# UzL-ITS/dash

Measured on AMD Instinct MI355X. Metric: online garbled inferences/sec (MiniONN CIFAR-10 CNN), higher is better.
Workload: dtype uint8 label components / int8 MFMA (exact modular arithmetic)

## Files before the change

dash_amd/csrc/hip/kernels_gadget.hip:

```cpp
#include <cmath>
#include <cstdio>
#include <cstdlib>

#include "gadget_common.h"

namespace dash {
namespace dev {


template <int TM>
__device__ __forceinline__ void approx_casts_out(const AesCtx& aes, const SignArgs& a, const ModC* mc, int j, int b,
                                                 int64_t e, const u128 (&P)[TM], const u128* TA, uint32_t col, u128 H) {
    const int64_t N = a.N;
    const int t = a.t;
    u128* out = a.mrsP + (static_cast<int64_t>(b) * a.crt.k + j) * t * N + e;
    if (a.fused) {
#pragma unroll
        for (int d = 0; d < TM; ++d)
            if (d < t) out[static_cast<int64_t>(d) * N] = P[d];
        for (int d = TM; d < t; ++d) out[static_cast<int64_t>(d) * N] = TA[col * t + d] - H;
        return;
    }
    const u128* T1 = a.cast1 + (static_cast<int64_t>(b) * N + e) * a.n_cast;
    out[0] = P[0];
// ... 1032 lines not shown
#pragma unroll
            for (int u = 0; u < kChunk; ++u)
                if (i0 + kChunk + u < n) nxt[u] = L[static_cast<int64_t>(i0 + kChunk + u) * N];
#pragma unroll
            for (int u = 0; u < kChunk; ++u)
                if (i0 + u < n) {
                    const uint32_t g = sg.next(m);
                    const uint32_t ev = se.next(m);
                    Y[static_cast<int64_t>(i0 + u) * N] =
                        static_cast<act_t>(modq(ev + ypr * static_cast<uint32_t>(cur[u]) + static_cast<uint32_t>(p) - g, m));
                }
#pragma unroll
            for (int u = 0; u < kChunk; ++u) cur[u] = nxt[u];
        }
    }
}

constexpr int kRroBS = 256;
__global__ __launch_bounds__(kRroBS) void k_rescale_relu_out_s(MrsArgs a, SignArgs sa, Act x, Act y, const u128* gtab,
                                                                const u128* etab, const ModC* mc, const uint32_t* te0,
                                                                const uint32_t* rk) {
    (void)te0;
    (void)rk;
    __shared__ __attribute__((aligned(16))) uint8_t stg[128 * kRroBS];
    const int j = blockIdx.y, b = blockIdx.z;
    const int64_t N = a.N;
    const int k = a.crt.k;
    const int p = a.crt.p[j];
    const ModC m = mc[p];
    const int n = static_cast<int>(m.n);
    const int tid = static_cast<int>(threadIdx.x);
    const uint32_t inv = static_cast<uint32_t>(a.sinv[j]);
    act_t* L = x.p[j] + static_cast<int64_t>(b) * n * N;
    act_t* Y = y.p[j] + static_cast<int64_t>(b) * n * N;
    for (int64_t e0 = static_cast<int64_t>(blockIdx.x) * kRroBS; e0 < N; e0 += static_cast<int64_t>(gridDim.x) * kRroBS) {
        const int64_t e = min(e0 + tid, N - 1);
        const int64_t be = static_cast<int64_t>(b) * N + e;
        const int64_t bke = (static_cast<int64_t>(b) * k + j) * N + e;
        const u128 HS = a.ys[(static_cast<int64_t>(b) * a.ny + j) * N + e];
        const u128 HM = a.ys[(static_cast<int64_t>(b) * a.ny + k + j / 8) * N + e] >> (16 * (j % 8));
        const uint32_t cS = a.cs[be];
        const u128* E3 = etab + (be * k + j) * 3;
        const u128 Eraw = E3[cS];
        const u128 mini = E3[2];
        const u128* grow = gtab + be * sa.crt.sum + sa.crt.prefix[j];
        const u128 P = a.pf[bke];
        __syncthreads();
        if (j != 0) lds_stage_rows<kRroBS, 4>(stg, L, N, e0, 0, n);
        __syncthreads();
        DigitStream s;
        s.init(P);
        CompressFwd cf;
        cf.init();
        u128 Graw = 0;
        constexpr int kRroG = 8;
        if (j == 0 && m.bits == 1) {
            Graw = grow[static_cast<uint32_t>(P) & 1u];
#pragma unroll
            for (int w = 0; w < 4; ++w) {
                const uint32_t pw = static_cast<uint32_t>(P >> (32 * w));
#pragma unroll 8
                for (int u = 0; u < 32; ++u) {
                    const int c = 32 * w + u;
                    if (c >= n) break;
                    stg[c * kRroBS + tid] = static_cast<uint8_t>((pw >> u) & 1u);
                }
            }
        }
        for (int c0 = 0; c0 < ((j == 0 && m.bits == 1) ? 0 : n); c0 += kRroG) {
            uint32_t w8[kRroG];
#pragma unroll
            for (int u = 0; u < kRroG; ++u) w8[u] = (j != 0 && c0 + u < n) ? stg[(c0 + u) * kRroBS + tid] : 0u;
#pragma unroll
            for (int u = 0; u < kRroG; ++u) {
                const int c = c0 + u;
                if (c >= n) break;
                const uint32_t v = j == 0 ? s.next(m) : modq(w8[u] * inv + s.next(m), m);
                if (c == 0) Graw = grow[v];
                stg[c * kRroBS + tid] = static_cast<uint8_t>(v);
                if (j != 0) cf.push(v, m);
            }
        }
        const u128 key = j == 0 ? P : cf.finish();
        __syncthreads();
        lds_store_rows<kRroBS>(L, stg, N, e0, 0, n);
        const u128 G = Graw - hard_pad(key, a.rgate0 ^ static_cast<uint64_t>(e), tw_sub(kTwMmg, j), 0);
        const u128 E = Eraw - HS;
        const int16_t t16 = static_cast<int16_t>(static_cast<uint16_t>(mini >> (16 * cS)));
        const int16_t ypr16 = static_cast<int16_t>(t16 - static_cast<int16_t>(static_cast<uint16_t>(HM)));
        const uint32_t ypr = modq(static_cast<uint32_t>(static_cast<int32_t>(ypr16) + (p << 15)), m);
        DigitStream sg, se;
        sg.init(G);
        se.init(E);
        __syncthreads();
        if (m.bits == 1) {
#pragma unroll
            for (int w = 0; w < 4; ++w) {
                const uint32_t ge = static_cast<uint32_t>(G >> (32 * w)) ^ static_cast<uint32_t>(E >> (32 * w));
#pragma unroll 8
                for (int u = 0; u < 32; ++u) {
                    const int c = 32 * w + u;
                    if (c >= n) break;
                    uint8_t& v = stg[c * kRroBS + tid];
                    v = static_cast<uint8_t>(((ge >> u) & 1u) ^ (static_cast<uint32_t>(v) & ypr));
                }
            }
        }
        for (int c0 = 0; c0 < (m.bits == 1 ? 0 : n); c0 += kRroG) {
            uint32_t w8[kRroG];
#pragma unroll
            for (int u = 0; u < kRroG; ++u) w8[u] = c0 + u < n ? stg[(c0 + u) * kRroBS + tid] : 0u;
#pragma unroll
            for (int u = 0; u < kRroG; ++u) {
                const int c = c0 + u;
                if (c >= n) break;
                const uint32_t g = sg.next(m);
                const uint32_t ev = se.next(m);
                stg[c * kRroBS + tid] = static_cast<uint8_t>(modq(ev + ypr * w8[u] + static_cast<uint32_t>(p) - g, m));
            }
        }
        __syncthreads();
        lds_store_rows<kRroBS>(Y, stg, N, e0, 0, n);
    }
}

constexpr int kRroQE = 64;
__device__ __forceinline__ void quad_stage_rows(uint8_t* S, const act_t* L, int64_t N, int64_t e0, int n) {
    if (N % 16 == 0) {
        for (int xu = threadIdx.x; xu < n * (kRroQE / 16); xu += blockDim.x) {
            const int row = xu / (kRroQE / 16), part = xu % (kRroQE / 16);
            const int64_t ee = e0 + 16 * part;
            if (ee < N) *reinterpret_cast<uint4*>(S + row * kRroQE + 16 * part) =
                *reinterpret_cast<const uint4*>(L + static_cast<int64_t>(row) * N + ee);
        }
    } else {
        for (int xb = threadIdx.x; xb < n * kRroQE; xb += blockDim.x) {
            const int row = xb / kRroQE, c = xb % kRroQE;
            if (e0 + c < N) S[xb] = L[static_cast<int64_t>(row) * N + e0 + c];
        }
    }
}
__device__ __forceinline__ void quad_store_rows(act_t* L, const uint8_t* S, int64_t N, int64_t e0, int n) {
    if (N % 16 == 0) {
        for (int xu = threadIdx.x; xu < n * (kRroQE / 16); xu += blockDim.x) {
            const int row = xu / (kRroQE / 16), part = xu % (kRroQE / 16);
            const int64_t ee = e0 + 16 * part;
            if (ee < N) *reinterpret_cast<uint4*>(L + static_cast<int64_t>(row) * N + ee) =
                *reinterpret_cast<const uint4*>(S + row * kRroQE + 16 * part);
        }
    } else {
        for (int xb = threadIdx.x; xb < n * kRroQE; xb += blockDim.x) {
            const int row = xb / kRroQE, c = xb % kRroQE;
            if (e0 + c < N) L[static_cast<int64_t>(row) * N + e0 + c] = S[xb];
        }
    }
}
static inline bool out_quad_fits(const MrsArgs& a, int B) {
    static const int mode = [] {
        const char* e = std::getenv("DASH_RRO_QUAD");
        return e ? std::atoi(e) : 1;
    }();
    bool fits = mode != 0 && (mode == 2 || (a.N + 255) / 256 * a.crt.k * B <= num_cus());
    for (int j = 0; j < a.crt.k; ++j) fits = fits && a.crt.n[j] <= 128;
    return fits;
}
__global__ __launch_bounds__(256) void k_rescale_relu_out_q(MrsArgs a, SignArgs sa, Act x, Act y, const u128* gtab,
                                                           const u128* etab, const ModC* mc) {
    __shared__ __attribute__((aligned(16))) uint8_t sL[128 * kRroQE];
    __shared__ __attribute__((aligned(16))) uint8_t sO[128 * kRroQE];
    const int j = blockIdx.y, b = blockIdx.z;
    const int64_t N = a.N;
    const int k = a.crt.k;
    const int p = a.crt.p[j];
    const ModC m = mc[p];
    const int n = static_cast<int>(m.n);
    const uint32_t q = m.q;
    const int tid = static_cast<int>(threadIdx.x);
    const int el = tid >> 2, g = tid & 3;
    const uint32_t inv = static_cast<uint32_t>(a.sinv[j]);
    act_t* L = x.p[j] + static_cast<int64_t>(b) * n * N;
    act_t* Yo = y.p[j] + static_cast<int64_t>(b) * n * N;
    for (int64_t e0 = static_cast<int64_t>(blockIdx.x) * kRroQE; e0 < N; e0 += static_cast<int64_t>(gridDim.x) * kRroQE) {
        const int64_t e = min(e0 + el, N - 1);
        const int64_t be = static_cast<int64_t>(b) * N + e;
        const int64_t bke = (static_cast<int64_t>(b) * k + j) * N + e;
        const u128 HS = a.ys[(static_cast<int64_t>(b) * a.ny + j) * N + e];
        const u128 HM = a.ys[(static_cast<int64_t>(b) * a.ny + k + j / 8) * N + e] >> (16 * (j % 8));
        const uint32_t cS = a.cs[be];
        const u128* E3 = etab + (be * k + j) * 3;
        const u128 mini = E3[2];
        const u128* grow = gtab + be * sa.crt.sum + sa.crt.prefix[j];
        const u128 P = a.pf[bke];
        const u128 Eraw = E3[cS];
        __syncthreads();
        if (j != 0) quad_stage_rows(sL, L, N, e0, n);
        __syncthreads();
        u128 Graw;
        {
            uint32_t pd0;
            if (m.bits) {
                pd0 = static_cast<uint32_t>(P) & (q - 1);
            } else {
                u128 t = P;
                uint32_t r = divmod128(t, m);
                pd0 = chunk_digit(r, m);
            }
// ... 9 lines not shown
                const int idx = g * cpl + t;
                if (idx >= n) break;
                const uint32_t pd = static_cast<uint32_t>(Pw >> (bb * t)) & (q - 1);
                const uint32_t v = j == 0 ? pd : modq(static_cast<uint32_t>(sL[idx * kRroQE + el]) * inv + pd, m);
                sL[idx * kRroQE + el] = static_cast<uint8_t>(v);
                part |= static_cast<u128>(v) << (bb * idx);
            }
        } else {
            pw.init(m);
            const int c = static_cast<int>(m.c), nch = (n + c - 1) / c;
            u128 Q = P, PW = pw.first(g);
            for (int jj = 0; 4 * jj < nch; ++jj) {
                uint32_t mine = 0;
#pragma unroll
                for (int u = 0; u < 4; ++u) {
                    if (4 * jj + u >= nch) break;
                    const uint32_t r = divmod128(Q, m);
                    mine = u == g ? r : mine;
                }
                const int i = 4 * jj + g;
                uint32_t cv = 0, pt = 1;
                for (int t = 0; t < c; ++t) {
                    const int idx = i * c + t;
                    const uint32_t pd = chunk_digit(mine, m);
                    if (idx < n) {
                        const uint32_t v = j == 0 ? pd : modq(static_cast<uint32_t>(sL[idx * kRroQE + el]) * inv + pd, m);
                        sL[idx * kRroQE + el] = static_cast<uint8_t>(v);
                        cv += v * pt;
                    }
                    pt *= q;
                }
                part += PW * static_cast<u128>(cv);
                PW *= pw.d4;
            }
        }
        const u128 key = j == 0 ? P : quad_sum128(part);
        u128 G;
        if constexpr (kQCoop) {
            uint32_t w[4];
            hard_block_q(key, a.rgate0 ^ static_cast<uint64_t>(e), tw_sub(kTwMmg, j), 0u, g, w);
            G = Graw - quad_gather128(w[0]);
        } else {
            G = Graw - hard_pad(key, a.rgate0 ^ static_cast<uint64_t>(e), tw_sub(kTwMmg, j), 0);
        }
        const u128 E = Eraw - HS;
        const int16_t t16 = static_cast<int16_t>(static_cast<uint16_t>(mini >> (16 * cS)));
        const int16_t ypr16 = static_cast<int16_t>(t16 - static_cast<int16_t>(static_cast<uint16_t>(HM)));
        const uint32_t ypr = modq(static_cast<uint32_t>(static_cast<int32_t>(ypr16) + (p << 15)), m);
        if (m.bits) {
            const uint64_t Gw = static_cast<uint64_t>(G >> (bb * g * cpl)), Ew = static_cast<uint64_t>(E >> (bb * g * cpl));
            for (int t = 0; t < cpl; ++t) {
                const int idx = g * cpl + t;
                if (idx >= n) break;
                const uint32_t gd = static_cast<uint32_t>(Gw >> (bb * t)) & (q - 1);
                const uint32_t ed = static_cast<uint32_t>(Ew >> (bb * t)) & (q - 1);
                sO[idx * kRroQE + el] =
                    static_cast<uint8_t>(modq(ed + ypr * static_cast<uint32_t>(sL[idx * kRroQE + el]) + static_cast<uint32_t>(p) - gd, m));
            }
        } else {
            const int c = static_cast<int>(m.c), nch = (n + c - 1) / c;
            u128 QG = G, QE = E;
            for (int jj = 0; 4 * jj < nch; ++jj) {
                uint32_t mg = 0, me = 0;
#pragma unroll
                for (int u = 0; u < 4; ++u) {
                    if (4 * jj + u >= nch) break;
                    const uint32_t rg = divmod128(QG, m);
                    const uint32_t re = divmod128(QE, m);
                    mg = u == g ? rg : mg;
                    me = u == g ? re : me;
                }
                const int i = 4 * jj + g;
                for (int t = 0; t < c; ++t) {
                    const int idx = i * c + t;
                    const uint32_t gd = chunk_digit(mg, m);
                    const uint32_t ed = chunk_digit(me, m);
                    if (idx < n)
                        sO[idx * kRroQE + el] = static_cast<uint8_t>(
                            modq(ed + ypr * static_cast<uint32_t>(sL[idx * kRroQE + el]) + static_cast<uint32_t>(p) - gd, m));
                }
            }
        }
        __syncthreads();
        quad_store_rows(L, sL, N, e0, n);
        quad_store_rows(Yo, sO, N, e0, n);
    }
}

void launch_rescale_relu_out(const MrsArgs& a, const SignArgs& sa, const Act& x, const Act& y, const u128* gtab,
                             const u128* etab, int B, const ModC* mc, const AesGlobals& g, hipStream_t st) {
    static const bool rro_stage = [] {
        const char* e = std::getenv("DASH_RRO_STAGE");
        return !(e && e[0] == '0');
    }();
    if (out_quad_fits(a, B)) {
        const dim3 gq(static_cast<unsigned>((a.N + kRroQE - 1) / kRroQE), a.crt.k, B);
        if (launch_log_on()) launch_log_add("relu_out.quad", gq, dim3(256));
        hipLaunchKernelGGL(k_rescale_relu_out_q, gq, dim3(256), 0, st, a, sa, x, y, gtab, etab, mc);
        return;
    }
    if (rro_stage && stage_ok(a.N, kRroBS)) {
        const dim3 gs(static_cast<unsigned>((a.N + kRroBS - 1) / kRroBS), a.crt.k, B);
        if (launch_log_on()) launch_log_add("relu_out.staged", gs, dim3(kRroBS));
        hipLaunchKernelGGL(k_rescale_relu_out_s, gs, dim3(kRroBS), 0, st, a, sa, x, y, gtab, etab, mc, g.te0, g.rk);
        return;
    }
    const LaunchDims d = aes_dims("relu_out.lane", a.N, a.crt.k, B);
    hipLaunchKernelGGL(k_rescale_relu_out, d.grid, d.block, kAesLds, st, a, sa, x, y, gtab, etab, mc, g.te0, g.rk);
}

__global__ __launch_bounds__(kAesBlock, kAesMinBlocks) void k_label_hash(Act x, CrtInfo crt, int64_t N, u128* hx,
                                                                        uint16_t* colx, const ModC* mc,
                                                                        const uint32_t* te0, const uint32_t* rk,
                                                                        int hard, uint64_t mgate0) {
    AES_PROLOGUE(te0, rk);
    const int j = blockIdx.y, b = blockIdx.z;
    for (int64_t e = static_cast<int64_t>(blockIdx.x) * blockDim.x + threadIdx.x; e < N;
         e += static_cast<int64_t>(gridDim.x) * blockDim.x) {
        const ModC m = mc[crt.p[j]];
        const act_t* L = x.p[j] + static_cast<int64_t>(b) * m.n * N + e;
        const int64_t bke = (static_cast<int64_t>(b) * crt.k + j) * N + e;
        colx[bke] = static_cast<uint16_t>(static_cast<uint16_t>(L[0]) % m.q);
        const u128 C = compress_cm(L, N, m);
        hx[bke] = hard ? hard_pad(C, mgate0 ^ static_cast<uint64_t>(e), tw_sub(kTwMmg, j), 0) : aes_encrypt(aes, C);
    }
}

static void dispatch_mrs_chain(const MrsArgs& a, const Act& x, int B, const ModC* mc, const AesGlobals& g,
                               hipStream_t st) {
    switch (a.crt.k) {
        case 2: launch_mrs_chain_k<2>(a, x, B, mc, g, st); break;
        case 3: launch_mrs_chain_k<3>(a, x, B, mc, g, st); break;
        case 4: launch_mrs_chain_k<4>(a, x, B, mc, g, st); break;
        case 5: launch_mrs_chain_k<5>(a, x, B, mc, g, st); break;
        case 6: launch_mrs_chain_k<6>(a, x, B, mc, g, st); break;
        case 7: launch_mrs_chain_k<7>(a, x, B, mc, g, st); break;
        case 8: launch_mrs_chain_k<8>(a, x, B, mc, g, st); break;
        case 9: launch_mrs_chain_k<9>(a, x, B, mc, g, st); break;
        case 10: launch_mrs_chain_k<10>(a, x, B, mc, g, st); break;
        case 11: launch_mrs_chain_k<11>(a, x, B, mc, g, st); break;
        case 12: launch_mrs_chain_k<12>(a, x, B, mc, g, st); break;
        default: std::fprintf(stderr, "dash: mixed-radix chains support 2..12 CRT residues\n"); std::abort();
    }
}

void launch_relu_mrs(const MrsArgs& a, const SignArgs& sa, const Act& x, const Act& y, const u128* gtab,
                     const u128* etab, int B, const ModC* mc, const AesGlobals& g, hipStream_t st) {
    AES_LAUNCH_GGL(k_label_hash, a.N, a.crt.k, B, kAesLds, st, x, a.crt, a.N, sa.hx, sa.colx, mc, g.te0, g.rk,
                   sa.hard, sa.mgate0);
    dispatch_mrs_chain(a, x, B, mc, g, st);
    launch_relu_mult(sa, x, y, gtab, etab, mc, st);
}

void launch_relu_joint(const SignArgs& sa, const Act& x, const Act& y, const u128* gtab, const u128* etab, int B,
                       const ModC* mc, const AesGlobals& g, hipStream_t st) {
    (void)B;
    (void)g;
    launch_relu_mult(sa, x, y, gtab, etab, mc, st);
}

__global__ __launch_bounds__(256) void k_rescale_mrs_out_q(MrsArgs a, Act x, const ModC* mc) {
    __shared__ __attribute__((aligned(16))) uint8_t sL[128 * kRroQE];
    const int j = blockIdx.y, b = blockIdx.z;
    const int64_t N = a.N;
    const int k = a.crt.k;
    const ModC m = mc[a.crt.p[j]];
    const int n = static_cast<int>(m.n);
    const uint32_t q = m.q;
    const int tid = static_cast<int>(threadIdx.x);
    const int el = tid >> 2, g = tid & 3;
    const uint32_t inv = static_cast<uint32_t>(a.sinv[j]);
    act_t* L = x.p[j] + static_cast<int64_t>(b) * n * N;
    for (int64_t e0 = static_cast<int64_t>(blockIdx.x) * kRroQE; e0 < N; e0 += static_cast<int64_t>(gridDim.x) * kRroQE) {
        const int64_t e = min(e0 + el, N - 1);
        const u128 P = a.pf[(static_cast<int64_t>(b) * k + j) * N + e];
        __syncthreads();
        if (j != 0) quad_stage_rows(sL, L, N, e0, n);
        __syncthreads();
        if (m.bits) {
            const int bb = static_cast<int>(m.bits), cpl = (n + 3) >> 2;
            const uint64_t Pw = static_cast<uint64_t>(P >> (bb * g * cpl));
// ... 296 lines not shown
```

dash_amd/csrc/hip/launch.h:

```cpp
#pragma once

#include <hip/hip_runtime.h>

#include <algorithm>
#include <atomic>
#include <cstdlib>
#include <map>
#include <mutex>
#include <string>
#include <vector>

#include "kargs.h"

namespace dash {
namespace dev {

int num_cus();
void set_planning_cus(int n);
int planning_cus_override();
extern std::atomic<bool> g_launch_log_on;
inline bool launch_log_on() { return g_launch_log_on.load(std::memory_order_relaxed); }
void launch_log_enable(bool on);
void launch_log_add(const std::string& form, dim3 grid, dim3 block);
std::vector<std::string> launch_log_take();


void launch_sign_approx(const SignArgs& a, const Act& x, const ModC* mc, const AesGlobals& g, hipStream_t st);
void launch_sign_chain(const SignArgs& a, int maxn, const ModC* mc, const AesGlobals& g, hipStream_t st);
void launch_unpack(const u128* P, int nres, const Act& out, const CrtInfo& mods, const ModC* mc, int64_t N, int B,
                   hipStream_t st);
void launch_clip_hash(const ClipArgs& a, u128* hx, uint16_t* colx, const Act& x, int B, const ModC* mc,
                      const AesGlobals& g, hipStream_t st);
void launch_clip_sign_mrs(const MrsArgs& a, const Act& x, int B, const ModC* mc, const AesGlobals& g, hipStream_t st);
void launch_clip_mult(const ClipArgs& a, const Act& x, const Act& y, int B, const ModC* mc, hipStream_t st);
void launch_relu_mult(const SignArgs& a, const Act& x, const Act& y, const u128* gtab, const u128* etab,
                      const ModC* mc, hipStream_t st);
void launch_rescale_hash(const Act& x, int fi, int s, const int16_t* up, int up_stride, int add_up, int64_t N, int B,
                         u128* h0, uint16_t* col0, const ModC* mc, const AesGlobals& g, hipStream_t st, int hard = 0);
void launch_rescale_update(const RescaleArgs& a, const Act& x, int B, const ModC* mc, hipStream_t st);
void launch_rescale_post(const Act& x, const CrtInfo& crt, int64_t N, int B, const u128* signP, const int16_t* down,
                         int lab_stride, const int* lab_off, const ModC* mc, hipStream_t st);
void launch_rescale_hash_sign(const u128* signP, const u128* du, int64_t N, int B, u128* h0, uint16_t* col0,
                              const AesGlobals& g, hipStream_t st);
void launch_rescale_update_approx(const RescaleArgs& r, const SignArgs& a, const Act& x, const int16_t* delta,
                                  const u128* zh, int B, const ModC* mc, const AesGlobals& g, hipStream_t st);
void launch_rescale_mrs(const MrsArgs& a, const Act& x, int B, const ModC* mc, const AesGlobals& g, hipStream_t st,
                        bool chain_only = false);
template <int K>
void launch_mrs_chain_k(const MrsArgs& a, const Act& x, int B, const ModC* mc, const AesGlobals& g, hipStream_t st);
void launch_rescale_relu_out(const MrsArgs& a, const SignArgs& sa, const Act& x, const Act& y, const u128* gtab,
                             const u128* etab, int B, const ModC* mc, const AesGlobals& g, hipStream_t st);
void launch_relu_joint(const SignArgs& sa, const Act& x, const Act& y, const u128* gtab, const u128* etab, int B,
                       const ModC* mc, const AesGlobals& g, hipStream_t st);
void launch_relu_mrs(const MrsArgs& a, const SignArgs& sa, const Act& x, const Act& y, const u128* gtab,
                     const u128* etab, int B, const ModC* mc, const AesGlobals& g, hipStream_t st);
void launch_base_ext(const BEArgs& a, const Act& x, int B, const ModC* mc, const AesGlobals& g, hipStream_t st);
void launch_proj(const ProjArgs& a, const Act& x, const Act& y, int B, const ModC* mc, const AesGlobals& g,
                 hipStream_t st);
void launch_mult(const MultArgs& a, const Act& x, const Act& y, int B, const ModC* mc, const AesGlobals& g,
                 hipStream_t st);

void launch_copy_gather(const Act& in, int64_t Nin, const Act& out, int64_t Nout, const int64_t* idx,
                        const CrtInfo& crt, int B, hipStream_t st);
void launch_pair_diff(const Act& v, int64_t Nv, const Act& d, int64_t Nout, int ops, int cnt, const CrtInfo& crt, int B,
                      hipStream_t st);
void launch_pair_add(const Act& v, int64_t Nv, const Act& r, const Act& nv, int64_t Nout, int ops, int cnt, int cnt1,
                     const CrtInfo& crt, int B, hipStream_t st);
void launch_add(const Act& x, const Act& y, int64_t N, const CrtInfo& crt, int B, hipStream_t st);
void launch_window_sum(const Act& in, int64_t Nin, const Act& out, int64_t Nout, const int64_t* idx, int K,
                       const CrtInfo& crt, int B, hipStream_t st);
struct PoolArgs {
    int C, H, W, kh, kw, sh, sw, ph, pw, OH, OW;
};
void launch_pool_sum(const Act& in, const Act& out, const PoolArgs& g, const CrtInfo& crt, int B, hipStream_t st);
void launch_concat_copy(const Act& src, int64_t Ns, const Act& out, int64_t Nout, int64_t off, const CrtInfo& crt,
                        int B, hipStream_t st);
void launch_aes_bench(u128* out, int blocks, int iters, const AesGlobals& g, hipStream_t st);
void launch_aes_test(const u128* in, u128* out, int64_t n, const AesGlobals& g, hipStream_t st);
void launch_hard_test(const u128* key, const uint64_t* gate, const uint32_t* sub, const uint32_t* blk, u128* out,
                      int64_t n, hipStream_t st);
void launch_codec_test(const int16_t* labels, int64_t N, int q, const ModC* mc, u128* comp, int16_t* decomp,
                       hipStream_t st);

struct DenseArgs {
    CrtInfo crt;
    int64_t K, O;
    const int16_t* w[kMaxRes];
    const int32_t* zc[kMaxRes];
    const int16_t* bias[kMaxRes];
    const int16_t* zero;
    int lab_stride;
    int lab_off[kMaxRes];
    const int32_t* src;
    const int8_t* w8[kMaxRes];
    int Kpad;
};
void launch_dense(const DenseArgs& a, const Act& x, const Act& y, int B, hipStream_t st);
void prepare_zmap(const CrtInfo& crt);

struct ConvArgs {
    CrtInfo crt;
    int C, H, W, F, kh, kw, sh, sw, ph, pw, OH, OW;
// ... 257 lines not shown
```

dash_amd/csrc/hip/runtime.hip:

```cpp
#include <pybind11/numpy.h>
#include <pybind11/pybind11.h>
#include <pybind11/stl.h>

#include <atomic>
#include <cstring>
#include <tuple>
#include <chrono>
#include <map>
#include <mutex>
#include <functional>
#include <thread>

#include "../layers.h"
#include "host_util.h"
#include "launch.h"
#include "fetch.h"

#include <rocprofiler-sdk-roctx/roctx.h>

namespace py = pybind11;

namespace dash {
using namespace dev;

// ... 1069 lines not shown
                        a.mode = 1;
                        a.hs = hs_;
                        a.cs = cs_;
                        a.gate0 = sgate;
                        a.rgate0 = ca.mgate0;
                        a.ny = 0;
                        a.ys = ys_;
                        a.ks = ks_[side];
                        add_op(lname + "." + pre + "mrs", [a, x, B, mc, ag](hipStream_t st) {
                            launch_clip_sign_mrs(a, x, B, mc, ag, st);
                        });
                    } else {
                        SignPlan sp(crt_, m0.h.mrs, {2}, 0, 1, m0.h.sign_fused != 0);
                        SignArgs a = make_sign(li, pre, sp, N, 0, sgate, 0);
                        a.outP = ks_[side];
                        if (side == 0) {
                            a.hx = hx_;
                            a.colx = colx_;
                            a.mgate0 = ca.mgate0;
                        }
                        const int maxn = sign_maxn_;
                        add_op(lname + "." + pre + "A", [a, x, mc, ag](hipStream_t st) { launch_sign_approx(a, x, mc, ag, st); });
                        add_op(lname + "." + pre + "B", [a, maxn, mc, ag](hipStream_t st) { launch_sign_chain(a, maxn, mc, ag, st); });
                    }
                }
                add_op(lname + ".C", [ca, x, y, B, mc](hipStream_t st) { launch_clip_mult(ca, x, y, B, mc, st); });
                cur = nxt;
                break;
            }
            case K_SIGN: {
                SignPlan sp(crt_, m0.h.mrs, crt_, -1, 1, m0.h.sign_fused != 0);
                SignArgs a = make_sign(li, "", sp, N, 0, gate_base(li + 1, 1), 0);
                Act x = act_of(cur), y = act_of(nxt);
                const ModC* mc = mc_;
                const AesGlobals ag = aes_;
                const int maxn = sign_maxn_;
                const int B = B_;
                const u128* outP = outP_;
                const i64 NN = N;
                add_op(lname + ".A", [a, x, mc, ag](hipStream_t st) { launch_sign_approx(a, x, mc, ag, st); });
                add_op(lname + ".B", [a, maxn, mc, ag](hipStream_t st) { launch_sign_chain(a, maxn, mc, ag, st); });
                add_op(lname + ".unpack", [outP, y, crt, mc, NN, B](hipStream_t st) { launch_unpack(outP, crt.k, y, crt, mc, NN, B, st); });
                cur = nxt;
                break;
            }
            case K_RESCALE: {
                const i64 mode = g.param("mode", 0);
                const i64 iters = g.param("iters");
                if (mode == 2) {
                    const bool so = g.param("sign_out", 0) == 1;
                    const RescaleMrsPlan P(crt_, static_cast<int>(g.param("l")), so);
                    DASH_CHECK(P.T <= m0.h.max_mod, "model lacks the mod-2^(l+1) label constants");
                    MrsArgs a{};
                    a.crt = crt;
                    a.T = static_cast<int>(P.T);
                    a.N = N;
                    a.n_tab = P.n_tab;
                    a.tab = upload_tables(li, "mrs");
                    for (int i = 0; i < k_; ++i) {
                        a.dig_off[i] = P.dig_off[i];
                        a.sinv[i] = static_cast<int>(P.Sinv[i]);
                    }
                    a.fin_off = P.fin_off;
                    const int bits = P.l + 1, nf = nr_comps(static_cast<int>(P.T));
                    a.hmask = 0;
                    for (int f = 0; f < nf; ++f) a.hmask |= static_cast<u128>(1) << (bits * f + bits - 1);
                    a.pf = outP_;
                    if (!mrs_ps_) mrs_ps_ = dalloc<u128>(static_cast<size_t>(B_) * std::max(1, k_ * (k_ - 1) / 2) * maxSignN_);
                    a.ps = mrs_ps_;
                    a.mode = so ? 2 : 0;
                    a.hs = hs_;
                    a.cs = cs_;
                    a.hx = hx_;
                    a.colx = colx_;
                    DASH_CHECK(hard_, "the mixed-radix rescale exists in the hardened encoding only");
                    a.gate0 = gate_base(li + 1, 30);
                    a.rgate0 = so ? gate_base(li + 2, 2) : 0;
                    a.ny = ny_;
                    a.ys = ys_;
                    Act x = act_of(cur);
                    const ModC* mc = mc_;
                    const AesGlobals ag = aes_;
                    const int B = B_;
                    static const int fuse_env = [] {
                        const char* e = std::getenv("DASH_JOINT_FUSE");
                        return e ? std::atoi(e) : -1;
                    }();
                    const bool fuse = fuse_env >= 0 ? fuse_env == 1 : B_ <= 2;
                    const bool defer = fuse && so && li + 1 < m0.layers.size() && m0.layers[li + 1].kind == K_RELU &&
                                       m0.layers[li + 1].param("smode", 0) == 2 && !keep[li + 1] &&
                                       !m0.layers[li + 1].p.count("in_src");
                    if (defer) {
                        joint_a_ = a;
                        joint_pending_ = true;
                    }
                    add_op(lname + ".mrs", [a, x, B, mc, ag, defer](hipStream_t st) {
                        launch_rescale_mrs(a, x, B, mc, ag, st, defer);
                    });
                    break;
                }
                if (mode == 0) {
                    plan_rescale_legacy(li, iters, N, crt, lname);
                    break;
                }
                for (i64 it = 0; it < iters; ++it) {
                    std::vector<int> factors;
                    if (mode == 0)
                        factors = {2};
                    else
                        for (auto v : g.vec("s")) factors.push_back(static_cast<int>(v));
                    RescalePlan P(crt_, m0.h.mrs, factors, mode == 0, m0.h.sign_fused != 0);
                    const std::string pre = arr_name("it", static_cast<int>(it), ".");
                    const u128* trans = upload_tables(li, pre + "trans");
                    Act x = act_of(cur);
                    const ModC* mc = mc_;
                    const AesGlobals ag = aes_;
                    const int B = B_;
                    const i64 NN = N;
                    i64 off = 0;
                    for (size_t f = 0; f < P.factors.size(); ++f) {
                        const int fi = P.factor_idx[f], s = P.factors[f];
                        const int add_up = f == 0 ? 1 : 0;
                        const int16_t* up = up_rows_ + lab_off_[fi];
                        u128* h0 = h0_;
                        uint16_t* col0 = col0_;
                        const int ls = lab_stride_;
                        const int hd = hard_ ? 1 : 0;
                        add_op(lname + ".hash", [x, fi, s, up, ls, add_up, NN, B, h0, col0, mc, ag, hd](hipStream_t st) {
                            launch_rescale_hash(x, fi, s, up, ls, add_up, NN, B, h0, col0, mc, ag, st, hd);
                        });
                        RescaleArgs ra{};
                        ra.crt = crt;
                        ra.N = N;
                        ra.fi = fi;
                        ra.s = s;
                        ra.add_up = add_up;
                        for (size_t q = 0; q < P.active[f].size(); ++q) {
                            const int jj = P.active[f][q];
                            ra.active[jj] = 1;
                            ra.aidx[jj] = static_cast<int>(q);
                            ra.inv[jj] = static_cast<int>(P.inv[f][q]);
                        }
                        ra.n_trans = P.n_trans;
                        ra.off = off;
                        off += static_cast<i64>(P.active[f].size()) * s;
                        ra.trans = trans;
                        ra.h0 = h0_;
                        ra.col0 = col0_;
                        ra.up = up_rows_;
                        ra.zero = zero_rows_;
                        ra.lab_stride = lab_stride_;
                        for (int j = 0; j < k_; ++j) ra.lab_off[j] = lab_off_[j];
                        ra.hard = hard_ ? 1 : 0;
                        ra.gate0 = gate_base(li + 1, 10 + it);
                        ra.factor = static_cast<int>(f);
                        add_op(lname + ".update", [ra, x, B, mc](hipStream_t st) { launch_rescale_update(ra, x, B, mc, st); });
                    }
                    const u128* signP = nullptr;
                    if (P.sign_be) {
                        SignArgs a = make_sign(li, pre, P.sign, N, 0);
                        const int maxn = sign_maxn_;
                        add_op(lname + ".sA", [a, x, mc, ag](hipStream_t st) { launch_sign_approx(a, x, mc, ag, st); });
                        add_op(lname + ".sB", [a, maxn, mc, ag](hipStream_t st) { launch_sign_chain(a, maxn, mc, ag, st); });
                        signP = outP_;
                    } else {
                        const BEPlan& be = P.be;
                        BEArgs ba{};
                        ba.E = static_cast<int>(be.moduli.size());
                        ba.nonext = be.nonext;
                        std::vector<int> idx(ba.E);
                        for (int i = 0; i < ba.E; ++i) idx[be.pos_of[i]] = i;
// ... 482 lines not shown
        out.append(py::make_tuple(x.p, arr));
    }
    return out;
}
CrtLabels labels_from_py2(const py::list& l) {
    CrtLabels out;
    for (auto item : l) {
        py::tuple t = item.cast<py::tuple>();
        int p = t[0].cast<int>();
        auto arr = py::array_t<int16_t, py::array::c_style | py::array::forcecast>::ensure(t[1]);
        DASH_CHECK(arr && arr.ndim() == 2, "labels must be (N, n) int16 arrays");
        Labels L(p, arr.shape(0));
        DASH_CHECK(arr.shape(1) == L.n, "label width does not match modulus");
        std::memcpy(L.c.data(), arr.data(), L.c.size() * sizeof(comp_t));
        out.push_back(std::move(L));
    }
    return out;
}
hipStream_t as_stream(uintptr_t s) { return reinterpret_cast<hipStream_t>(s); }
}

void register_guard_bindings(py::module_& m);

void register_hip_bindings(py::module_& m) {
    register_guard_bindings(m);
    m.def("encode_compressed_into", [](const Garbler& g, py::array_t<i64, py::array::c_style | py::array::forcecast> x,
                                       HipEvaluator& h, int b) {
        DASH_CHECK(x.size() == h.input_size(), "input size mismatch");
        u128* dst = h.input_slot_compressed(b);
        const i64* xp = x.data();
        const i64 N = x.size();
        py::gil_scoped_release rel;
        g.encode_compressed(xp, N, dst);
    });
    py::class_<DeviceInputEncoder>(m, "DeviceInputEncoder")
        .def(py::init<const Garbler&, int, int, int>(), py::arg("garbler"), py::arg("device"), py::arg("slots") = 1,
             py::arg("slot") = 0)
        .def("input_size", &DeviceInputEncoder::input_size)
        .def("slots", &DeviceInputEncoder::slots)
        .def("load", &DeviceInputEncoder::load, py::arg("garbler"), py::arg("slot") = 0,
             py::call_guard<py::gil_scoped_release>())
        .def("encode_into", [](DeviceInputEncoder& enc, HipEvaluator& h, int b0,
                               py::array_t<i64, py::array::c_style | py::array::forcecast> x, uintptr_t stream) {
            const int n = x.ndim() == 2 ? static_cast<int>(x.shape(0)) : 1;
            const i64 N = x.ndim() == 2 ? static_cast<i64>(x.shape(1)) : static_cast<i64>(x.size());
            DASH_CHECK(x.ndim() == 1 || x.ndim() == 2, "DeviceInputEncoder: x must be (N,) or (slots, N)");
            enc.encode(h, b0, x.data(), n, N, as_stream(stream));
        }, py::arg("evaluator"), py::arg("slot"), py::arg("x"), py::arg("stream") = 0);
    m.def("encode_into", [](const Garbler& g, py::array_t<i64, py::array::c_style | py::array::forcecast> x,
                            HipEvaluator& h, int b) {
        auto slot = h.input_slot(b);
        DASH_CHECK(x.size() == h.input_size(), "input size mismatch");
        const i64* xp = x.data();
        const i64 N = x.size();
        py::gil_scoped_release rel;
        g.encode_cm(xp, N, slot);
    });
    m.def("hip_stream_create", [](int priority) {
        hipStream_t st = nullptr;
        HIPCHECK(hipStreamCreateWithPriority(&st, hipStreamNonBlocking, priority));
        return reinterpret_cast<uintptr_t>(st);
    }, py::arg("priority") = 0);
    m.def("hip_stream_destroy", [](uintptr_t st) { HIPCHECK(hipStreamDestroy(reinterpret_cast<hipStream_t>(st))); });
    m.def("hip_stream_sync", [](uintptr_t st) { HIPCHECK(hipStreamSynchronize(reinterpret_cast<hipStream_t>(st))); });
    m.def("hip_stream_wait", [](uintptr_t st, double timeout_s) {
        py::gil_scoped_release rel;
        const auto t0 = std::chrono::steady_clock::now();
        for (int spin = 0;; ++spin) {
            const hipError_t e = hipStreamQuery(reinterpret_cast<hipStream_t>(st));
            if (e == hipSuccess) return true;
            if (e != hipErrorNotReady) HIPCHECK(e);
            const double dt = std::chrono::duration<double>(std::chrono::steady_clock::now() - t0).count();
            if (timeout_s >= 0 && dt > timeout_s) return false;
            if (spin > 64) std::this_thread::sleep_for(std::chrono::microseconds(spin > 4096 ? 1000 : 50));
        }
    }, py::arg("stream"), py::arg("timeout_s"));
    m.def("hip_clear_last_error", []() { return static_cast<int>(hipGetLastError()); });
    m.def("hip_set_planning_cus", [](int n) {
        DASH_CHECK(n >= 0, "hip_set_planning_cus: n must be >= 0 (0 restores the device's count)");
        dev::set_planning_cus(n);
    }, py::arg("n"));
    m.def("hip_planning_cus", []() { return dev::num_cus(); });
    m.def("hip_planning_override", []() { return dev::planning_cus_override(); });
    m.def("hip_launch_log", [](bool on) { dev::launch_log_enable(on); }, py::arg("on"));
    m.def("hip_launch_log_take", []() { return dev::launch_log_take(); });
    m.def("hip_conv_plan", [](int C, int H, int W, int F, int kh, int kw, int sh, int sw, int ph, int pw,
                              const std::vector<int>& crt_moduli, bool mfma) {
        DASH_CHECK(C > 0 && H > 0 && W > 0 && F > 0 && kh > 0 && kw > 0 && sh > 0 && sw > 0 && ph >= 0 && pw >= 0,
                   "hip_conv_plan: bad conv geometry");
        DASH_CHECK(!crt_moduli.empty() && static_cast<int>(crt_moduli.size()) <= dev::kMaxRes,
                   "hip_conv_plan: 1 .. 16 CRT moduli");
        dev::ConvArgs a{};
        a.crt.k = static_cast<int>(crt_moduli.size());
        for (int j = 0; j < a.crt.k; ++j) {
            DASH_CHECK(crt_moduli[j] >= 2, "hip_conv_plan: modulus below 2");
            a.crt.p[j] = crt_moduli[j];
            a.crt.n[j] = nr_comps(crt_moduli[j]);
        }
        a.C = C; a.H = H; a.W = W; a.F = F; a.kh = kh; a.kw = kw; a.sh = sh; a.sw = sw; a.ph = ph; a.pw = pw;
        a.OH = (H + 2 * ph - kh) / sh + 1;
        a.OW = (W + 2 * pw - kw) / sw + 1;
        DASH_CHECK(a.OH > 0 && a.OW > 0, "hip_conv_plan: empty output");
        dev::conv_layer_plan(a, mfma && dev::conv_img_enabled());
        py::dict d;
        d["ur"] = a.ur;
        d["KS"] = a.kh * a.kw * (a.Cpad / 64);
        d["Cpad"] = a.Cpad;
        d["Kpad"] = a.Kpad;
        d["ldsS"] = a.ldsS;
        d["ldsR"] = a.ldsR;
        d["band"] = a.band;
        d["nbands"] = a.nbands;
        d["OH"] = a.OH;
        d["OW"] = a.OW;
        d["sh24"] = std::vector<int>(a.sh24, a.sh24 + a.crt.k);
        return d;
    }, py::arg("C"), py::arg("H"), py::arg("W"), py::arg("F"), py::arg("kh"), py::arg("kw"), py::arg("sh"),
       py::arg("sw"), py::arg("ph"), py::arg("pw"), py::arg("crt_moduli"), py::arg("mfma") = true);
    m.def("hip_device_count", []() {
        int n = 0;
        if (hipGetDeviceCount(&n) != hipSuccess) return 0;
        return n;
    });
    m.def("hip_device_pci_bus_id", [](int device) {
        char buf[64] = {0};
        HIPCHECK(hipDeviceGetPCIBusId(buf, static_cast<int>(sizeof(buf)), device));
        return std::string(buf);
    });
    py::class_<IpcTables, std::shared_ptr<IpcTables>>(m, "IpcTables")
        .def(py::init([](int device, const py::list& handles, int B) {
                 std::vector<std::tuple<size_t, std::string, size_t, std::string>> hs;
                 for (auto item : handles) {
                     auto t = item.cast<py::tuple>();
                     hs.emplace_back(t[0].cast<size_t>(), t[1].cast<std::string>(), t[2].cast<size_t>(),
                                     t[3].cast<std::string>());
                 }
                 return std::make_shared<IpcTables>(device, hs, B);
             }),
             py::arg("device"), py::arg("handles"), py::arg("batch"))
        .def("tables", &IpcTables::tables)
        .def("sink", &IpcTables::sink, "slot b of the evaluator's table arenas as a GPU-garbler destination");
    py::class_<HipEvaluator, std::shared_ptr<HipEvaluator>>(m, "HipEvaluator")
        .def(py::init([](std::shared_ptr<GarbledModel> tmpl, int B, int device, bool mfma, bool stream_tables) {
                 return std::make_shared<HipEvaluator>(std::move(tmpl), B, device, mfma, stream_tables);
             }),
             py::arg("template"), py::arg("batch"), py::arg("device") = 0, py::arg("mfma") = true,
             py::arg("stream_tables") = false)
        .def_property_readonly("streams_tables", &HipEvaluator::streams_tables)
        .def("load", [](HipEvaluator& h, int b, std::shared_ptr<GarbledModel> m) {
            py::gil_scoped_release rel;
            h.load(b, *m);
        })
        .def("sink", &HipEvaluator::sink, "slot b's table arenas as a GPU-garbler destination (zero-copy load)")
        .def("ipc_export", [](const HipEvaluator& h) {
            py::list out;
            for (const auto& e : h.ipc_export())
                out.append(py::make_tuple(std::get<0>(e), std::get<1>(e), std::get<2>(e), py::bytes(std::get<3>(e))));
            return out;
        }, "IPC handles of the table arenas: [(layer, table, bytes per slot, handle)] (same-node device transport)")
        .def_property_readonly("batch", &HipEvaluator::batch)
        .def("device_bytes", &HipEvaluator::device_bytes)
        .def("table_bytes", &HipEvaluator::table_bytes)
        .def("set_profile", &HipEvaluator::set_profile)
        .def("op_times", &HipEvaluator::op_times)
        .def("set_inputs", [](HipEvaluator& h, const py::list& inputs, uintptr_t stream) {
            std::vector<CrtLabels> in;
// ... 159 lines not shown
```

Before: 3271.

## Add throughput relu_out kernel for large batches and widen joint-fuse selection

Measured after the change: 3822 (median of 6 runs). +16.9%, better.

```diff
diff --git a/dash_amd/csrc/hip/kernels_gadget.hip b/dash_amd/csrc/hip/kernels_gadget.hip
--- a/dash_amd/csrc/hip/kernels_gadget.hip
+++ b/dash_amd/csrc/hip/kernels_gadget.hip
@@ -1138,8 +1138,6 @@
             }
         }
         const u128 key = j == 0 ? P : cf.finish();
-        __syncthreads();
-        lds_store_rows<kRroBS>(L, stg, N, e0, 0, n);
         const u128 G = Graw - hard_pad(key, a.rgate0 ^ static_cast<uint64_t>(e), tw_sub(kTwMmg, j), 0);
         const u128 E = Eraw - HS;
         const int16_t t16 = static_cast<int16_t>(static_cast<uint16_t>(mini >> (16 * cS)));
@@ -1148,7 +1146,6 @@
         DigitStream sg, se;
         sg.init(G);
         se.init(E);
-        __syncthreads();
         if (m.bits == 1) {
 #pragma unroll
             for (int w = 0; w < 4; ++w) {
@@ -1178,6 +1175,130 @@
         __syncthreads();
         lds_store_rows<kRroBS>(Y, stg, N, e0, 0, n);
     }
+}
+
+constexpr int kRrtBS = 256;
+constexpr int kRrtCap = 80;
+static inline bool rrt_fits(const MrsArgs& a) {
+    bool fits = a.crt.p[0] == 2 && a.crt.n[0] <= 128;
+    for (int j = 1; j < a.crt.k; ++j) fits = fits && (a.crt.p[j] & (a.crt.p[j] - 1)) != 0 && a.crt.n[j] <= kRrtCap;
+    return fits;
+}
+__device__ __forceinline__ void rrt_stage_rows(uint8_t* S, const act_t* L, int64_t N, int64_t e0, int cnt) {
+    constexpr int W = kRrtBS / 16;
+    const int units = cnt * W;
+    auto ld = [=](int xu) {
+        const int64_t e = e0 + 16 * (xu % W);
+        uint4 v = make_uint4(0u, 0u, 0u, 0u);
+        if (xu < units && e < N) v = *reinterpret_cast<const uint4*>(L + static_cast<int64_t>(xu / W) * N + e);
+        return v;
+    };
+    auto st = [=](int xu, uint4 v) {
+        if (xu < units) *reinterpret_cast<uint4*>(S + (xu / W) * kRrtBS + 16 * (xu % W)) = v;
+    };
+    for (int x0 = threadIdx.x; x0 < units; x0 += 4 * kRrtBS) {
+        const uint4 v0 = ld(x0), v1 = ld(x0 + kRrtBS), v2 = ld(x0 + 2 * kRrtBS), v3 = ld(x0 + 3 * kRrtBS);
+        st(x0, v0);
+        st(x0 + kRrtBS, v1);
+        st(x0 + 2 * kRrtBS, v2);
+        st(x0 + 3 * kRrtBS, v3);
+    }
+}
+__global__ __launch_bounds__(kRrtBS) void k_rescale_relu_out_t(MrsArgs a, SignArgs sa, Act x, Act y, const u128* gtab,
+                                                                const u128* etab, const ModC* mc) {
+    __shared__ __attribute__((aligned(16))) uint8_t stg[kRrtCap * kRrtBS];
+    const int j = blockIdx.y, b = blockIdx.z;
+    const int64_t N = a.N;
+    const int k = a.crt.k;
+    const int p = a.crt.p[j];
+    const ModC m = mc[p];
+    const int n = static_cast<int>(m.n);
+    const int tid = static_cast<int>(threadIdx.x);
+    const int64_t e0 = static_cast<int64_t>(blockIdx.x) * kRrtBS;
+    const int64_t e = min(e0 + tid, N - 1);
+    const int64_t be = static_cast<int64_t>(b) * N + e;
+    const act_t* L = x.p[j] + static_cast<int64_t>(b) * n * N;
+    act_t* Y = y.p[j] + static_cast<int64_t>(b) * n * N;
+    const u128 P = a.pf[(static_cast<int64_t>(b) * k + j) * N + e];
+    const u128 HS = a.ys[(static_cast<int64_t>(b) * a.ny + j) * N + e];
+    const u128 HM = a.ys[(static_cast<int64_t>(b) * a.ny + k + j / 8) * N + e] >> (16 * (j % 8));
+    const uint32_t cS = a.cs[be];
+    const u128* E3 = etab + (be * k + j) * 3;
+    const u128 Eraw = E3[cS];
+    const u128 mini = E3[2];
+    const u128* grow = gtab + be * sa.crt.sum + sa.crt.prefix[j];
+    const uint64_t gate = a.rgate0 ^ static_cast<uint64_t>(e);
+    if (j == 0) {
+        const u128 Graw = grow[static_cast<uint32_t>(P) & 1u];
+        const u128 G = Graw - hard_pad(P, gate, tw_sub(kTwMmg, 0), 0);
+        const u128 E = Eraw - HS;
+        const uint32_t t16 = static_cast<uint32_t>(mini >> (16 * cS)), hm = static_cast<uint32_t>(HM);
+        const u128 R = (G ^ E) ^ (((t16 ^ hm) & 1u) ? P : static_cast<u128>(0));
+        for (int q0 = 0; q0 < n; q0 += kRrtCap) {
+            const int cnt = min(kRrtCap, n - q0);
+            if (q0) __syncthreads();
+            const u128 Rw = R >> q0;
+#pragma unroll
+            for (int w = 0; w < (kRrtCap + 31) / 32; ++w) {
+                const uint32_t rw = static_cast<uint32_t>(Rw >> (32 * w));
+#pragma unroll 8
+                for (int u = 0; u < 32; ++u) {
+                    const int c = 32 * w + u;
+                    if (c >= cnt) break;
+                    stg[c * kRrtBS + tid] = static_cast<uint8_t>((rw >> u) & 1u);
+                }
+            }
+            __syncthreads();
+            lds_store_rows<kRrtBS>(Y, stg, N, e0, q0, cnt);
+        }
+        return;
+    }
+    const uint32_t inv = static_cast<uint32_t>(a.sinv[j]);
+    const int c = static_cast<int>(m.c);
+    rrt_stage_rows(stg, L, N, e0, n);
+    __syncthreads();
+    u128 Graw;
+    {
+        u128 t = P;
+        uint32_t r = divmod128(t, m);
+        const uint32_t pd0 = chunk_digit(r, m);
+        Graw = grow[modq(static_cast<uint32_t>(stg[tid]) * inv + pd0, m)];
+    }
+    u128 Q = P, C = 0, PW = 1;
+    for (int k0 = 0; k0 < n; k0 += c) {
+        uint32_t r = divmod128(Q, m);
+        const int kc = min(c, n - k0);
+        uint32_t acc = 0, pt = 1;
+#pragma unroll 4
+        for (int t = 0; t < kc; ++t) {
+            uint8_t& w = stg[(k0 + t) * kRrtBS + tid];
+            const uint32_t v = modq(static_cast<uint32_t>(w) * inv + chunk_digit(r, m), m);
+            w = static_cast<uint8_t>(v);
+            acc += v * pt;
+            pt *= m.q;
+        }
+        C += PW * static_cast<u128>(acc);
+        PW *= static_cast<u128>(m.D);
+    }
+    const u128 G = Graw - hard_pad(C, gate, tw_sub(kTwMmg, j), 0);
+    const u128 E = Eraw - HS;
+    const int16_t t16 = static_cast<int16_t>(static_cast<uint16_t>(mini >> (16 * cS)));
+    const int16_t ypr16 = static_cast<int16_t>(t16 - static_cast<int16_t>(static_cast<uint16_t>(HM)));
+    const uint32_t ypr = modq(static_cast<uint32_t>(static_cast<int32_t>(ypr16) + (p << 15)), m);
+    u128 QG = G, QE = E;
+    for (int k0 = 0; k0 < n; k0 += c) {
+        uint32_t rg = divmod128(QG, m), re = divmod128(QE, m);
+        const int kc = min(c, n - k0);
+#pragma unroll 4
+        for (int t = 0; t < kc; ++t) {
+            const uint32_t g = chunk_digit(rg, m);
+            const uint32_t ev = chunk_digit(re, m);
+            uint8_t& v = stg[(k0 + t) * kRrtBS + tid];
+            v = static_cast<uint8_t>(modq(ev + ypr * static_cast<uint32_t>(v) + static_cast<uint32_t>(p) - g, m));
+        }
+    }
+    __syncthreads();
+    lds_store_rows<kRrtBS>(Y, stg, N, e0, 0, n);
 }
 
 constexpr int kRroQE = 64;
@@ -1353,9 +1474,26 @@
             }
         }
         __syncthreads();
-        quad_store_rows(L, sL, N, e0, n);
         quad_store_rows(Yo, sO, N, e0, n);
     }
+}
+
+static std::atomic<int>& joint_fuse_state() {
+    static std::atomic<int> mode{[] {
+        const char* e = std::getenv("DASH_JOINT_FUSE");
+        const int v = e ? std::atoi(e) : -1;
+        return v > 0 ? 1 : (v == 0 ? 0 : -1);
+    }()};
+    return mode;
+}
+int joint_fuse_mode() { return joint_fuse_state().load(std::memory_order_relaxed); }
+void set_joint_fuse(int mode) { joint_fuse_state().store(mode > 0 ? 1 : (mode == 0 ? 0 : -1), std::memory_order_relaxed); }
+constexpr int64_t kJointFuseMinElems = 24 * 576;
+int64_t joint_fuse_min_elems() { return kJointFuseMinElems; }
+bool joint_fuse_pick(int64_t N, int B) { return B <= 2 || (stage_ok(N, kRrtBS) && B * N >= kJointFuseMinElems); }
+bool joint_fuse(int64_t N, int B) {
+    const int mode = joint_fuse_mode();
+    return mode >= 0 ? mode == 1 : joint_fuse_pick(N, B);
 }
 
 void launch_rescale_relu_out(const MrsArgs& a, const SignArgs& sa, const Act& x, const Act& y, const u128* gtab,
@@ -1368,6 +1506,12 @@
         const dim3 gq(static_cast<unsigned>((a.N + kRroQE - 1) / kRroQE), a.crt.k, B);
         if (launch_log_on()) launch_log_add("relu_out.quad", gq, dim3(256));
         hipLaunchKernelGGL(k_rescale_relu_out_q, gq, dim3(256), 0, st, a, sa, x, y, gtab, etab, mc);
+        return;
+    }
+    if (rro_stage && B >= 3 && stage_ok(a.N, kRrtBS) && rrt_fits(a)) {
+        const dim3 gt(static_cast<unsigned>((a.N + kRrtBS - 1) / kRrtBS), a.crt.k, B);
+        if (launch_log_on()) launch_log_add("relu_out.tput", gt, dim3(kRrtBS));
+        hipLaunchKernelGGL(k_rescale_relu_out_t, gt, dim3(kRrtBS), 0, st, a, sa, x, y, gtab, etab, mc);
         return;
     }
     if (rro_stage && stage_ok(a.N, kRroBS)) {
diff --git a/dash_amd/csrc/hip/launch.h b/dash_amd/csrc/hip/launch.h
--- a/dash_amd/csrc/hip/launch.h
+++ b/dash_amd/csrc/hip/launch.h
@@ -18,6 +18,11 @@
 int num_cus();
 void set_planning_cus(int n);
 int planning_cus_override();
+int64_t joint_fuse_min_elems();
+int joint_fuse_mode();
+void set_joint_fuse(int mode);
+bool joint_fuse_pick(int64_t N, int B);
+bool joint_fuse(int64_t N, int B);
 extern std::atomic<bool> g_launch_log_on;
 inline bool launch_log_on() { return g_launch_log_on.load(std::memory_order_relaxed); }
 void launch_log_enable(bool on);
diff --git a/dash_amd/csrc/hip/runtime.hip b/dash_amd/csrc/hip/runtime.hip
--- a/dash_amd/csrc/hip/runtime.hip
+++ b/dash_amd/csrc/hip/runtime.hip
@@ -1175,11 +1175,7 @@
                     const ModC* mc = mc_;
                     const AesGlobals ag = aes_;
                     const int B = B_;
-                    static const int fuse_env = [] {
-                        const char* e = std::getenv("DASH_JOINT_FUSE");
-                        return e ? std::atoi(e) : -1;
-                    }();
-                    const bool fuse = fuse_env >= 0 ? fuse_env == 1 : B_ <= 2;
+                    const bool fuse = dev::joint_fuse(N, B_);
                     const bool defer = fuse && so && li + 1 < m0.layers.size() && m0.layers[li + 1].kind == K_RELU &&
                                        m0.layers[li + 1].param("smode", 0) == 2 && !keep[li + 1] &&
                                        !m0.layers[li + 1].p.count("in_src");
@@ -1828,6 +1824,16 @@
     }, py::arg("n"));
     m.def("hip_planning_cus", []() { return dev::num_cus(); });
     m.def("hip_planning_override", []() { return dev::planning_cus_override(); });
+    m.def("hip_set_joint_fuse", [](int mode) {
+        DASH_CHECK(mode >= -1 && mode <= 1, "hip_set_joint_fuse: mode must be -1 (auto), 0 (off) or 1 (on)");
+        dev::set_joint_fuse(mode);
+    }, py::arg("mode"));
+    m.def("hip_joint_fuse", []() { return dev::joint_fuse_mode(); });
+    m.def("hip_joint_fuse_pick", [](int64_t N, int B) {
+        DASH_CHECK(N >= 1 && B >= 1, "hip_joint_fuse_pick: N and B must be positive");
+        return dev::joint_fuse_pick(N, B);
+    }, py::arg("N"), py::arg("B"));
+    m.def("hip_joint_fuse_min_elems", []() { return dev::joint_fuse_min_elems(); });
     m.def("hip_launch_log", [](bool on) { dev::launch_log_enable(on); }, py::arg("on"));
     m.def("hip_launch_log_take", []() { return dev::launch_log_take(); });
     m.def("hip_conv_plan", [](int C, int H, int W, int F, int kh, int kw, int sh, int sw, int ph, int pw,
```
